# double125/MADTP

Measured on AMD Instinct MI355X. Metric: images/sec forward, BLIP-base NLVR2 p=0.5 b64; pruned-token index match, higher is better.
Workload: dtype bf16

## Files before the change

include/madtp_hip.h:

```cpp
#ifndef MADTP_HIP_H
#define MADTP_HIP_H

#include <stddef.h>
#include <stdint.h>

#ifdef __cplusplus
extern "C" {
#endif

#define MADTP_F32 0
#define MADTP_BF16 1
#define MADTP_F16S 2
#define MADTP_F16 3

#define MADTP_E_BADARG (-1)
#define MADTP_E_SHAPE (-2)
#define MADTP_E_DTYPE (-3)
#define MADTP_E_ALIGN (-4)
#define MADTP_E_BUSY (-5)
#define MADTP_E_RANGE (-6)

#define MADTP_ACT_NONE 0
#define MADTP_ACT_GELU_ERF 1
#define MADTP_ACT_QUICK_GELU 2
// ... 185 lines not shown
    const float* self_mask_qk;
    int ld_self_mask_qk;
} madtp_bert_layer_w;

size_t madtp_bert_layer_workspace(int B, int L, int Nk, int dim, int hidden, int heads, int dtype);

int madtp_bert_layer_attn(const madtp_bert_layer_w* w, const float* hidden, const float* mask2d, float* att, void* ws,
                          size_t ws_bytes, int B, int L, int Nk, const float* token_attn, int ldt_row, int ldt_batch, int K,
                          float temperature, float* score, float* threshold, int32_t* count, int32_t* kmax, void* stream);

int madtp_bert_layer_rest(const madtp_bert_layer_w* w, const float* att, const float* mask2d, float* y, float* mask_out,
                          void* ws, size_t ws_bytes, int B, int L, int k, const float* score, int64_t* indices,
                          int64_t* indices_sort, int cross_mode, const void* enc0, const void* enc1, int Nk,
                          const float* enc_mask0, const float* enc_mask1, void* stream);

int madtp_bert_layer(const madtp_bert_layer_w* w, const float* hidden, const float* mask2d, float* att, float* y,
                     float* mask_out, void* ws, size_t ws_bytes, int B, int L, int Nk, const float* token_attn, int ldt_row,
                     int ldt_batch, int K, float temperature, float* score, float* threshold, int32_t* count,
                     int64_t* indices, int64_t* indices_sort, int cross_mode, const void* enc0, const void* enc1,
                     const float* enc_mask0, const float* enc_mask1, const void* hidden_lp, void* y_lp, const void* kv_pre0,
                     const void* kv_pre1, const int32_t* kv_index, int kv_ld, int* k_out, int* k_used, void* stream);

typedef struct madtp_query_w {
    const void* sd_w;
    const void* sd_hi; const void* sd_lo; int split_dtype; float sd_scale;
    int K; float inv_sqrt_sd;
    float* att_ft;
    float* stats_ws;
} madtp_query_w;

typedef struct madtp_layer_io {
    float* logits;
    float* x_attn;
    float* y;
    void* y_lp;
    float* mask_out;
    float* score; float* threshold; int32_t* count;
    int64_t* indices; int64_t* indices_sort;
    int k_out, k_used, n_out;
} madtp_layer_io;

int madtp_vit_encoder(const madtp_vit_block_w* const* layers, int n_layers, const madtp_query_w* q, const float* x0,
                      madtp_layer_io* io, void* ws, size_t ws_bytes, int B, int N0, float temperature, void* stream);

int madtp_vit_encoder_async(const madtp_vit_block_w* const* layers, int n_layers, const madtp_query_w* q, const float* x0,
                            madtp_layer_io* io, void* ws, size_t ws_bytes, int B, int N0, float temperature, int32_t* dims_dev,
                            int32_t* dims_host, void* stream);

int madtp_bert_encoder(const madtp_bert_layer_w* const* layers, int n_layers, const madtp_query_w* q, const float* hidden0,
                       const void* hidden0_lp, const float* mask0, madtp_layer_io* io, void* ws, size_t ws_bytes, int B, int L0,
                       int Nk, float temperature, int cross_mode, const void* enc0, const void* enc1, const float* enc_mask0,
                       const float* enc_mask1, const void* const* kv_pre0, const void* const* kv_pre1, const int32_t* kv_index,
                       int kv_ld, void* stream);

int madtp_bert_encoder_async(const madtp_bert_layer_w* const* layers, int n_layers, const madtp_query_w* q, const float* hidden0,
                             const void* hidden0_lp, const float* mask0, madtp_layer_io* io, void* ws, size_t ws_bytes, int B, int L0,
                             int Nk, float temperature, int cross_mode, const void* enc0, const void* enc1, const float* enc_mask0,
                             const float* enc_mask1, const void* const* kv_pre0, const void* const* kv_pre1, const int32_t* kv_index,
                             int kv_ld, int32_t* dims_dev, int32_t* dims_host, void* stream);

int madtp_bert_decode_step(const madtp_bert_layer_w* const* layers, int n_layers, const float* x, void* kv_cache, int rows, int t,
                           int Lmax, const void* const* kv_pre, const int32_t* kv_index, int kv_ld, int Nk, int group, float* y,
                           void* ws, size_t ws_bytes, void* stream);
int madtp_kv_cache_reorder(const void* src, void* dst, const int64_t* beam_src, int n_layers, int rows, int Lmax, int t, int row_bytes,
                           void* stream);

int madtp_lm_loss(const float* logits, int ld, int rows_per_seq, int n_pred, int V, const int64_t* labels, int ld_labels,
                  float label_smoothing, float* loss, int B, void* stream);
int madtp_token_prob(const float* logits, int ld, int V, const int64_t* tok, int A, float* out, int Q, void* stream);
int madtp_beam_topk(const float* logits, int ld, int V, const float* beam_scores, int num_beams, int n_top, int suppress_token,
                    float* out_scores, int32_t* out_index, int B, void* stream);
int madtp_beam_topk_penalty(const float* logits, int ld, int V, const float* beam_scores, int num_beams, int n_top,
                            int suppress_token, const int64_t* prev_ids, int ld_prev, int cur_len, float repetition_penalty,
                            float* out_scores, int32_t* out_index, int B, void* stream);
int madtp_beam_update(const float* cand_scores, const int32_t* cand_index, int n_top, int V, const int64_t* ids_in, int64_t* ids_out,
                      int ld_ids, int cur_len, float* beam_scores, int64_t* beam_src, int32_t* hyp_n, int32_t* hyp_order,
                      double* hyp_score, int32_t* hyp_len, int64_t* hyp_tok, double* worst, int32_t* done, int32_t* err, double denom,
                      int num_beams, int eos_token, int pad_token, int early_stopping, int B, void* stream);
int madtp_sample_top_p(const float* logits, int ld, int V, const int64_t* prev_ids, int ld_prev, int cur_len, float repetition_penalty,
                       int suppress_token, int top_k, float top_p, const float* u, int64_t* out_token, float* out_prob, int B,
                       void* stream);


int madtp_transpose_pad(const float* src, int ld_src, int R, int C, float* dst, int ld_dst, int Rp, int Cp, void* stream);
int madtp_transpose_split(const float* src, int ld_src, int R, int C, void* dst, int Rp, int Cp, int weight_format,
                          float* colsum_out, float* colsum_ws, void* stream);
int madtp_weight_planes(const float* w, int ldw, int N, int K, float inv_scale, void* planes, int row0, void* planes_t, int Ntp, int col0,
                        void* stream);
int madtp_colsum(const float* dy, int ld, int M, int N, float* out, float* part_ws, void* stream);
int madtp_act_fwd_bwd(const float* u, const float* dg, float* g, float* du, size_t n, int act, void* stream);
int madtp_layernorm_bwd(const float* x, const float* gamma, const float* dy, const float* add, float* dx, float* dgamma,
                        float* dbeta, float* ws, int rows, int dim, float eps, void* stream);
int madtp_token_gather_bwd(const float* dy, const float* x, const int32_t* dst_pos, const float* merge_w, float* dx, float* dw,
                           int B, int N, int k, int dim, void* stream);
int madtp_token_score_bwd(const float* dw, const float* score, const int32_t* dst_pos, const float* merge_w,
                          const float* colsum_part, int n_row_tiles, const float* p0, const float* onorm,
                          const float* token_attn, int ldt_row, int ldt_batch, int K, float* da, float* dp0, float* dnrm_scale,
                          float* dtoken_attn, int B, int H, int N, void* stream);
size_t madtp_attention_bwd_cross_workspace(int B, int H, int Nq, int Nk);
int madtp_attention_bwd_cross(const float* q, int ldq, const float* k, const float* v, int ldkv, const float* key_mask,
                              const float* dout, int ldo, float* dq, int lddq, float* dk, float* dv, int lddkv, void* ws,
                              size_t ws_bytes, int B, int H, int Nq, int Nk, float scale, float p_drop,
                              unsigned long long seed, unsigned long long site, void* stream);

int madtp_dropout(const float* x, const float* residual, float* y, size_t n, size_t per_sample, float p, unsigned long long seed,
                  unsigned long long site, void* stream);
// ... 36 lines not shown
```

madtp_amd/bert.py:

```python
import json
import math
import os

import torch
import torch.nn as nn

from . import hip
from .runtime import autograd_precision as _autograd_precision, EncoderWeights, PreparedCache, param_epoch, own_modules, get_precision, encoder_call_preference, f32_ptr, attn_dtype, compute_dtype, dtype_code, lin_of, require_gpu, as_f32_contig, to_compute
from .utils import Query_model


class BertConfig:
    _defaults = dict(vocab_size=30522, hidden_size=768, num_hidden_layers=12, num_attention_heads=12,
                     intermediate_size=3072, hidden_act="gelu", hidden_dropout_prob=0.1,
                     attention_probs_dropout_prob=0.1, max_position_embeddings=512, type_vocab_size=2,
                     initializer_range=0.02, layer_norm_eps=1e-12, pad_token_id=0, position_embedding_type="absolute",
                     add_cross_attention=False, encoder_width=768, chunk_size_feed_forward=0, evaluate=True,
                     output_attentions=False, output_hidden_states=False, use_return_dict=True, is_decoder=False)

    def __init__(self, **kw):
        for k, v in {**self._defaults, **kw}.items():
            setattr(self, k, v)

    @classmethod
# ... 554 lines not shown
    def _enc_mask2d(m):
        if m is None:
            return None
        return as_f32_contig(m[:, 0, 0, :]) if m.dim() == 4 else as_f32_contig(m)

    def feed_forward_chunk(self, attention_output):
        raise NotImplementedError("fused into forward()")


class MedBertLayer(_BertLayerBase):
    variant = "med"

    def forward(self, hidden_states, attention_mask=None, head_mask=None, encoder_hidden_states=None,
                encoder_attention_mask=None, past_key_value=None, output_attentions=False, mode=None, space_dict=None,
                token_attn=None, reduce_num=0, temperature=0):
        return self._forward(hidden_states, attention_mask, head_mask, encoder_hidden_states, encoder_attention_mask,
                             past_key_value, output_attentions, mode, token_attn, temperature)


class NlvrBertLayer(_BertLayerBase):
    variant = "nlvr"

    def forward(self, hidden_states, attention_mask=None, space_dict=None, head_mask=None, encoder_hidden_states=None,
                encoder_attention_mask=None, past_key_value=None, output_attentions=False, mode=None, token_attn=None,
                reduce_num=0, temperature=0):
        return self._forward(hidden_states, attention_mask, head_mask, encoder_hidden_states, encoder_attention_mask,
                             past_key_value, output_attentions, mode, token_attn, temperature)


class _Out(tuple):

    def __new__(cls, last_hidden_state):
        o = super().__new__(cls, (last_hidden_state,))
        o.last_hidden_state = last_hidden_state
        o.past_key_values = None
        o.hidden_states = None
        o.attentions = None
        o.cross_attentions = None
        o.pooler_output = None
        return o


class _BertEncoderBase(nn.Module):
    layer_cls = MedBertLayer

    def __init__(self, config, sd_dim=768):
        super().__init__()
        self.config = config
        self.layer = nn.ModuleList([self.layer_cls(config, i) for i in range(config.num_hidden_layers)])
        self.gradient_checkpointing = False
        self.txt_query_model = Query_model(ft_dim=config.hidden_size, sd_dim=sd_dim, temperature=1,
                                           att_func_type='sparsemax', pool_type='max')
        self._cache = PreparedCache()

    def _run(self, hidden_states, attention_mask, space_dict, temperature, encoder_hidden_states, encoder_attention_mask,
             mode, always_query):
        sd_txt_ft_all = None
        cache = self.__dict__.pop("_kv_cache", None)
        if torch.is_grad_enabled() and _autograd_precision() and cache is None:
            encs = [] if encoder_hidden_states is None else (list(encoder_hidden_states) if isinstance(encoder_hidden_states, (list, tuple))
                                                              else [encoder_hidden_states])
            if (hidden_states.requires_grad or (space_dict is not None and space_dict.requires_grad)
                    or any(e.requires_grad for e in encs) or any(p.requires_grad for p in self.parameters())):
                from .backward import bert_encoder_forward_with_grad
                self.__dict__.pop("_prepared_weights", None)
                h, _, sd_all = bert_encoder_forward_with_grad(self, hidden_states, attention_mask, space_dict, temperature,
                                                              encoder_hidden_states, encoder_attention_mask, mode, always_query)
                return _Out(h), sd_all
        if (_use_encoder_call(hidden_states.shape[0], _ENCODER_CALL) and not _KV_AHEAD
                and all(type(l) is self.layer_cls for l in self.layer)):
            out = self._run_encoder_call(hidden_states, attention_mask, space_dict, temperature, encoder_hidden_states,
                                         encoder_attention_mask, mode, always_query, cache)
            if out is not None:
                return out
        defer = self.txt_query_model.deferred() if space_dict is not None else None
        reduce_num = int((hidden_states.shape[-2] - 1) // self.config.num_hidden_layers)
        ahead = None
        if cache is None and mode == 'multimodal' and encoder_hidden_states is not None and _KV_AHEAD:
            ahead = self._project_encoder_tokens(encoder_hidden_states)
        for i, layer_module in enumerate(self.layer):
            layer_module.__dict__.pop("_kv_pre", None)
            if cache is not None and mode == 'multimodal':
                layer_module._kv_pre = (cache.kv[i], cache.Nk, cache.index)
            elif ahead is not None:
                kvs, Nk, width = ahead
                layer_module._kv_pre = (tuple(kv[:, i * width:(i + 1) * width] for kv in kvs) if len(kvs) == 2
                                        else kvs[0][:, i * width:(i + 1) * width], Nk, None)
            token_attn = None
            if space_dict is not None or always_query:
                if space_dict is None:
                    raise TypeError("nlvr_encoder.BertEncoder calls txt_query_model unconditionally (:608): "
                                    "space_dict must be given")
                token_attn, sd_txt_ft_all, _ = self.txt_query_model(hidden_states[:, 1:, :], space_dict,
                                                                    return_token_att=True, temperature=temperature,
                                                                    acc_ft=sd_txt_ft_all, defer=defer)
            t = temperature if space_dict is not None else 0
            if self.layer_cls.variant == "nlvr":
                outs = layer_module(hidden_states, attention_mask, space_dict, None, encoder_hidden_states,
                                    encoder_attention_mask, None, False, mode=mode, token_attn=token_attn,
                                    reduce_num=reduce_num, temperature=t)
            else:
                outs = layer_module(hidden_states, attention_mask, None, encoder_hidden_states, encoder_attention_mask,
                                    None, False, mode=mode, space_dict=space_dict, token_attn=token_attn,
                                    reduce_num=reduce_num, temperature=t)
            hidden_states = outs[0]
            attention_mask = outs[-1]
        if defer is not None and defer.pairs:
            sd_txt_ft_all = defer.finish()
        return _Out(hidden_states), sd_txt_ft_all


    def _run_options(self, hidden_states, attention_mask, head_mask, encoder_hidden_states, encoder_attention_mask, past_key_values,
                     use_cache, output_attentions, output_hidden_states, mode, space_dict, temperature, always_query):
        all_hidden = () if output_hidden_states else None
        all_self = () if output_attentions else None
        all_cross = () if (output_attentions and mode == 'multimodal') else None
        next_cache = () if use_cache else None
        sd_txt_ft_all = None
        require_gpu(hidden_states, "hidden_states")
        for i, layer_module in enumerate(self.layer):
            layer_module.__dict__.pop("_kv_pre", None)
            if output_hidden_states:
                all_hidden = all_hidden + (hidden_states,)
            token_attn = None
            if space_dict is not None or always_query:
                if space_dict is None:
                    raise TypeError("nlvr_encoder.BertEncoder calls txt_query_model unconditionally (:608): space_dict must be given")
                token_attn, sd_txt_ft_all, _ = self.txt_query_model(hidden_states[:, 1:, :], space_dict, return_token_att=True,
                                                                    temperature=temperature, acc_ft=sd_txt_ft_all)
            t = temperature if space_dict is not None else 0
            lhm = head_mask[i] if head_mask is not None else None
            hm = layer_module._head_mask_vec(lhm, hidden_states.device) if lhm is not None else None
            outs = layer_module._forward_general(as_f32_contig(hidden_states), attention_mask, hm, encoder_hidden_states,
                                                 encoder_attention_mask, past_key_values[i] if past_key_values is not None else None,
                                                 bool(output_attentions), mode, token_attn, t)
            hidden_states, attention_mask = outs[0], outs[-1]
            if use_cache:
                next_cache = next_cache + (outs[-2],)
            if output_attentions:
                all_self = all_self + (outs[1],)
                if all_cross is not None:
                    all_cross = all_cross + ((outs[2] if len(outs) == 5 else tuple(outs[2:-2])),)
        if output_hidden_states:
            all_hidden = all_hidden + (hidden_states,)
        out = _Out(hidden_states)
        out.past_key_values, out.hidden_states, out.attentions, out.cross_attentions = next_cache, all_hidden, all_self, all_cross
        return out, sd_txt_ft_all

    def _apply(self, fn, recurse=True):
        self.__dict__.pop("_enc_weights", None)
        return super()._apply(fn, recurse)

    def _encoder_weights(self):
        ew = self.__dict__.get("_enc_weights")
        if ew is None:
            ew = self.__dict__["_enc_weights"] = EncoderWeights()
        return ew.get(list(self.layer))

    def prepare_encoder_call(self, batch=None):
        if (batch is None or _use_encoder_call(batch, _ENCODER_CALL)) and _ENCODER_CALL and not _KV_AHEAD \
                and all(type(l) is self.layer_cls for l in self.layer):
            self.__dict__["_prepared_weights"] = (param_epoch(), get_precision(), self._encoder_weights())

    def _run_encoder_call(self, hidden_states, attention_mask, space_dict, temperature, encoder_hidden_states,
                          encoder_attention_mask, mode, always_query, cache):
        require_gpu(hidden_states, "hidden_states")
        query = space_dict is not None or always_query
        if query and space_dict is None:
            raise TypeError("nlvr_encoder.BertEncoder calls txt_query_model unconditionally (:608): space_dict must be given")
        hidden = as_f32_contig(hidden_states)
        B, L, D = hidden.shape
        mask2d = None
        if attention_mask is not None:
            if attention_mask.dim() == 4 and attention_mask.shape[2] == L and L > 1:
                return None
            if attention_mask.dim() != 4 or attention_mask.shape[2] != 1:
                raise NotImplementedError("only padding masks [B,1,1,L] and decoder masks [B,1,L,L] are supported")
            mask2d = as_f32_contig(attention_mask[:, 0, 0, :])
        t = temperature if space_dict is not None else 0
        if t > 0 and mask2d is None:
            raise ValueError("attention_mask is required when temperature > 0 (med.py:424)")
        qargs, deferred = (None, False)
        if query:
            qargs, deferred = self.txt_query_model.encoder_args(space_dict, B, D, hidden.device)
            if qargs is None:
                return None
        l0 = self.layer[0]
        cross = mode == 'multimodal'
        enc0 = enc1 = em0 = em1 = None
        kv0 = kv1 = kv_index = None
        Nk = 0
        nlvr = self.layer_cls.variant == "nlvr"
        if cross and cache is not None:
            Nk, kv0, kv_index = cache.Nk, list(cache.kv), cache.index
            if nlvr:
                return None
        elif cross:
            assert encoder_hidden_states is not None, "encoder_hidden_states must be given for cross-attention layers"
            if nlvr:
                Nk = encoder_hidden_states[0].shape[1]
                enc0, enc1 = l0._enc_operand(encoder_hidden_states[0]), l0._enc_operand(encoder_hidden_states[1])
                em0, em1 = l0._enc_mask2d(encoder_attention_mask[0]), l0._enc_mask2d(encoder_attention_mask[1])
            else:
                Nk = encoder_hidden_states.shape[1]
                enc0 = l0._enc_operand(encoder_hidden_states)
        lp = getattr(hidden_states, "_madtp_lp", None)
        if lp is not None and (lp[1] != hidden._version or hidden is not hidden_states or lp[0].shape[:-1] != hidden.shape[:-1]
                               or compute_dtype() == torch.float32 or lp[0].dtype != compute_dtype()):
            lp = None
        ws = self.__dict__.pop("_prepared_weights", None)
        if ws is not None and ws[:2] == (param_epoch(), get_precision()):
            ws = ws[2]
        else:
            ws = self._encoder_weights()
        kv_ld = 0
        if kv0 is not None:
            for tns in kv0:
                if tns.stride(-1) != 1 or (kv_ld and kv_ld != tns.stride(0)):
                    raise RuntimeError("encoder_kv_cache tensors must be row-major with one common row stride")
                kv_ld = tns.stride(0)
        from . import vit as _vit
        sync_free = _vit._SYNC_FREE and query and t > 0 and hip.bert_encoder_sync_free_ok(B, L, Nk, True, qargs, mask2d)
        run = hip.bert_encoder(ws, hidden, lp[0] if lp else None, mask2d, qargs, t, cross, enc0, enc1, Nk, em0, em1,
                               kv_pre0=kv0, kv_pre1=kv1, kv_index=kv_index, kv_ld=kv_ld, sync_free=sync_free)
        for l, layer in enumerate(self.layer):
            layer.last_prune = run.info(l, t if query else 0)
            layer.__dict__.pop("_kv_pre", None)
        sd_txt_ft_all = None
        qm = self.txt_query_model
        if query and qm.compute_att_ft:
            if deferred:
                K = space_dict.shape[0]
                segs = []
                for l in range(len(self.layer)):
                    n_in = run.n_in(l)
                    xp = hidden.data_ptr() if l == 0 else run.ptr(l - 1, "y")
                    segs.append((run.ptr(l, "logits") + 128 * 4, xp + D * 4, n_in - 1, 128, n_in * 128, D, n_in * D))
                sd_txt_ft_all = hip.query_att_ft_multi_ptrs(segs, B, K, D, hidden.device, sd_dim=qm.att_dim, exact={"exact": True, "split": "split"}.get(deferred, False))
            else:
                sd_txt_ft_all = qargs["att_ft"]
        self._last_run = run
        out = run.output(len(self.layer) - 1)
        if run.lp_dtype is not None:
            nl = len(self.layer) - 1
            out._madtp_lp = (run.view(nl, "y_lp", run.lp_dtype, B, out.shape[1], (2 * D if run.lp_dtype == torch.float16 else D)),
                             out._version)
        return _Out(out), sd_txt_ft_all

    def _project_encoder_tokens(self, encoder_hidden_states):
        encs = list(encoder_hidden_states) if isinstance(encoder_hidden_states, (list, tuple)) else [encoder_hidden_states]
        if not all(getattr(l, "has_cross", hasattr(l, "crossattention")) for l in self.layer):
            return None
        kvs = []
        for br, enc in enumerate(encs):
            mods = []
            for l in self.layer:
                ca = l.crossattention
                sm = (ca.self0, ca.self1)[br] if ca.twin else ca.self
                mods += [sm.key, sm.value]
            lin = lin_of(self._cache, ("kv_all", br), mods)
            kvs.append(hip.gemm(self.layer[0]._enc_operand(enc), lin.w, lin.b, n=lin.n, out_dtype=attn_dtype()))
        return kvs, encs[0].shape[1], 2 * self.config.hidden_size


class MedBertEncoder(_BertEncoderBase):
    layer_cls = MedBertLayer

    def forward(self, hidden_states, attention_mask=None, head_mask=None, encoder_hidden_states=None,
                encoder_attention_mask=None, past_key_values=None, use_cache=None, output_attentions=False,
                output_hidden_states=False, return_dict=True, mode='multimodal', space_dict=None, temperature=0):
        if head_mask is not None or past_key_values is not None or use_cache or output_attentions or output_hidden_states:
            return self._run_options(hidden_states, attention_mask, head_mask, encoder_hidden_states, encoder_attention_mask,
                                     past_key_values, use_cache, output_attentions, output_hidden_states, mode, space_dict,
                                     temperature, always_query=False)
        return self._run(hidden_states, attention_mask, space_dict, temperature, encoder_hidden_states,
                         encoder_attention_mask, mode, always_query=False)


class NlvrBertEncoder(_BertEncoderBase):
    layer_cls = NlvrBertLayer

    def forward(self, hidden_states, attention_mask=None, space_dict=None, temperature=0, head_mask=None,
                encoder_hidden_states=None, encoder_attention_mask=None, past_key_values=None, use_cache=None,
                output_attentions=False, output_hidden_states=False, return_dict=True, mode='multimodal'):
        if head_mask is not None or past_key_values is not None or use_cache or output_attentions or output_hidden_states:
            return self._run_options(hidden_states, attention_mask, head_mask, encoder_hidden_states, encoder_attention_mask,
                                     past_key_values, use_cache, output_attentions, output_hidden_states, mode, space_dict,
                                     temperature, always_query=True)
        return self._run(hidden_states, attention_mask, space_dict, temperature, encoder_hidden_states,
                         encoder_attention_mask, mode, always_query=True)


class _BertModelBase(nn.Module):
    encoder_cls = MedBertEncoder

    def __init__(self, config, add_pooling_layer=True, sd_dim=768):
        super().__init__()
        if add_pooling_layer:
            raise NotImplementedError("BLIP builds its text encoders with add_pooling_layer=False")
        self.config = config
        self.embeddings = BertEmbeddings(config)
        self.encoder = self.encoder_cls(config, sd_dim)
        self.pooler = None
        if not getattr(config, "evaluate", True):
            self.apply(self._init_weights)

    def _init_weights(self, module):
        if isinstance(module, (nn.Linear, nn.Embedding)):
            module.weight.data.normal_(mean=0.0, std=self.config.initializer_range)
        elif isinstance(module, nn.LayerNorm):
            module.bias.data.zero_()
            module.weight.data.fill_(1.0)
        if isinstance(module, nn.Linear) and module.bias is not None:
            module.bias.data.zero_()

# ... 367 lines not shown
```

madtp_amd/csrc/layers.hip:

```cpp
#include "common.h"
#include "internal.h"
#include <stdlib.h>

namespace {

struct Carver {
    char* base; size_t off; size_t cap;
    void* take(size_t bytes) {
        off = (off + 255) & ~(size_t)255;
        void* p = base ? base + off : nullptr;
        off += bytes;
        return p;
    }
    bool fits() const { return !base || off <= cap; }
};

inline size_t esz_of(int dt) { return (dt == MADTP_BF16 || dt == MADTP_F16) ? 2 : 4; }
inline int pld(int dt, int ld) { return dt == MADTP_F16S ? 2 * ld : ld; }
inline int attn_dt(int dt) { return dt == MADTP_F16S ? MADTP_F32 : dt; }
inline int attn_io(int dt) { return dt == MADTP_F16S ? MADTP_F16S : dt; }
inline int slabs_of(int K, int dt) { return dt == MADTP_F32 ? K / 32 : K / 64; }

#define TRY(call)                  \
    do {                           \
// ... 797 lines not shown
                                       (const char*)k1 + (size_t)D * e, (kv_pre0 && kv_pre0[l]) ? kv_index : nullptr, v.cat,
                                       (char*)v.cat + (size_t)D * e, em0, em1, B, w->heads, L0, Nk, 2 * D, ldkv, ldkv, 2 * D, w->scale,
                                       attn_io(dt), 0, dl + DIMS_STRIDE, stream));
            const void* catc = v.cat;
            if (dt == MADTP_F16S) {
                TRY(madtp_i_split_f16((const float*)v.cat, 2 * D, v.mid, 4 * D, Mmax, 2 * D, m_out, stream));
                catc = v.mid;
            }
            TRY(lin_ln_dev(catc, 2 * D, w->cdense_fused, a32, w->fused_twin == 2 ? 1.f : 0.5f, w->ln_cross_g, w->ln_cross_b, v.att2,
                           lpm ? v.attc : nullptr, Mmax, dt, w->eps, v.part, m_out, stream));
            a32 = v.att2;
            ac = lpm ? (const void*)v.attc : (const void*)v.att2;
        } else if (cross == 1) {
            TRY(lin_dev(ac, D, w->cq[0], nullptr, 0, v.q, D, Mmax, dt, adt, MADTP_ACT_NONE, m_out, stream));
            const void* k0 = kv_pre0 ? kv_pre0[l] : nullptr;
            int ldkv = 2 * D;
            if (!k0) {
                if (!enc0) return MADTP_E_BADARG;
                TRY(lin(enc0, D, w->ckv[0], nullptr, 0, v.kv, 2 * D, B * Nk, dt, adt, MADTP_ACT_NONE, 1.f, stream));
                k0 = v.kv;
            } else if (kv_ld) ldkv = kv_ld;
            TRY(madtp_i_attention_cross(v.q, k0, (const char*)k0 + (size_t)D * e, (kv_pre0 && kv_pre0[l]) ? kv_index : nullptr, v.c0,
                                        w->variant_nlvr ? enc_mask0 : nullptr, B, w->heads, L0, Nk, D, ldkv, ldkv, D, w->scale, attn_io(dt),
                                        dl + DIMS_STRIDE, stream));
            const void* cc = v.c0;
            if (dt == MADTP_F16S) {
                TRY(madtp_i_split_f16((const float*)v.c0, D, v.mid, 2 * D, Mmax, D, m_out, stream));
                cc = v.mid;
            }
            TRY(lin_ln_dev(cc, D, w->cdense[0], a32, 1.f, w->ln_cross_g, w->ln_cross_b, v.att2, lpm ? v.attc : nullptr, Mmax, dt, w->eps,
                           v.part, m_out, stream));
            a32 = v.att2;
            ac = lpm ? (const void*)v.attc : (const void*)v.att2;
        }
        TRY(lin_dev(ac, D, w->inter, nullptr, 0, v.mid, w->inter.n, Mmax, dt, dt, MADTP_ACT_GELU_ERF, m_out, stream));
        TRY(lin_ln_dev(v.mid, w->inter.n, w->out, a32, 1.f, w->ln_out_g, w->ln_out_b, o.y, lpm ? o.y_lp : nullptr, Mmax, dt, w->eps, v.part,
                       m_out, stream));
        h = o.y;
        h_lp = lpm ? o.y_lp : nullptr;
        mask = o.mask_out;
    }
    he = hipMemcpyAsync(dims_host, dims_dev, nrec * sizeof(int32_t), hipMemcpyDeviceToHost, s);
    if (he == hipSuccess) he = hipStreamSynchronize(s);
    if (he != hipSuccess) return (int)he;
    for (int l = 0; l < n_layers; ++l) {
        io[l].k_out = dims_host[l * DIMS_STRIDE + 1];
        io[l].k_used = dims_host[l * DIMS_STRIDE + 2];
        io[l].n_out = dims_host[l * DIMS_STRIDE + 3];
    }
    const int* rf = madtp_internal_range_flag();
    return (rf && *(const volatile int*)rf) ? MADTP_E_RANGE : 0;
}

extern "C" int madtp_bert_encoder(const madtp_bert_layer_w* const* layers, int n_layers, const madtp_query_w* q, const float* hidden0,
                                  const void* hidden0_lp, const float* mask0, madtp_layer_io* io, void* ws, size_t ws_bytes, int B,
                                  int L0, int Nk, float temperature, int cross_mode, const void* enc0, const void* enc1,
                                  const float* enc_mask0, const float* enc_mask1, const void* const* kv_pre0,
                                  const void* const* kv_pre1, const int32_t* kv_index, int kv_ld, void* stream) {
    if (!layers || !io || !hidden0 || n_layers <= 0 || B <= 0 || L0 <= 0) return MADTP_E_BADARG;
    const float* h = hidden0;
    const void* h_lp = hidden0_lp;
    const float* mask = mask0;
    int L = L0;
    const bool prune = q && temperature > 0.f;
    const int kp = q ? (q->K + 127) / 128 * 128 : 0;
    for (int l = 0; l < n_layers; ++l) {
        madtp_layer_io& o = io[l];
        const madtp_bert_layer_w* w = layers[l];
        if (!w || !o.x_attn || !o.y) return MADTP_E_BADARG;
        if (q) {
            if (!o.logits) return MADTP_E_BADARG;
            TRY(query_step(q, h, o.logits, l, B, L, w->dim, stream));
        }
        int k_out = 0, k_used = 0;
        const void* kv0 = kv_pre0 ? kv_pre0[l] : nullptr;
        const void* kv1 = kv_pre1 ? kv_pre1[l] : nullptr;
        if (prune)
            TRY(madtp_bert_layer(w, h, mask, o.x_attn, o.y, o.mask_out, ws, ws_bytes, B, L, Nk, o.logits + kp, kp, L * kp, q->K,
                                 temperature, o.score, o.threshold, o.count, o.indices, o.indices_sort, cross_mode, enc0, enc1,
                                 enc_mask0, enc_mask1, h_lp, o.y_lp, kv0, kv1, kv_index, kv_ld, &k_out, &k_used, stream));
        else
            TRY(madtp_bert_layer(w, h, mask, o.x_attn, o.y, nullptr, ws, ws_bytes, B, L, Nk, nullptr, 0, 0, 0, 0.f, nullptr, nullptr,
                                 nullptr, nullptr, nullptr, cross_mode, enc0, enc1, enc_mask0, enc_mask1, h_lp, o.y_lp, kv0, kv1,
                                 kv_index, kv_ld, &k_out, &k_used, stream));
        if (k_used > 0) {
            L = k_used + 2;
            if (mask) mask = o.mask_out;
        }
        o.k_out = k_out; o.k_used = k_used; o.n_out = L;
        h = o.y;
        h_lp = o.y_lp;
    }
    return 0;
}
```

madtp_amd/hip.py:

```python
import ctypes
import os
from ctypes import c_float, c_int, c_size_t, c_void_p

import torch

F32, BF16, F16S, F16 = 0, 1, 2, 3
ACT_NONE, ACT_GELU, ACT_QUICK_GELU, ACT_RELU = 0, 1, 2, 3
ABI_VERSION = 31

_HERE = os.path.dirname(os.path.abspath(__file__))
LIB_PATH = os.path.join(_HERE, "lib", "libmadtp_hip.so")

_SIGS = {
    "madtp_abi_version": (c_int, []),
    "madtp_strerror": (ctypes.c_char_p, [c_int]),
    "madtp_profile_begin": (c_int, []),
    "madtp_profile_end": (c_int, [ctypes.c_char_p, c_int]),
    "madtp_gemm": (c_int, [c_void_p] * 5 + [c_int] * 7 + [c_int, c_int, c_int, c_float, c_float, c_void_p]),
    "madtp_gemm_set_config": (c_int, [c_int]),
    "madtp_gemm_plan": (c_int, [c_int] * 11 + [c_void_p, c_void_p, c_int]),
    "madtp_stream_create_cumask": (c_int, [c_void_p, c_void_p, c_int]),
    "madtp_stream_set_sched": (c_int, [c_void_p, c_int, c_float, c_int]),
    "madtp_stream_get_sched": (c_int, [c_void_p, c_void_p, c_void_p, c_void_p]),
    "madtp_stream_destroy": (c_int, [c_void_p]),
# ... 2 lines not shown
    "madtp_splitk_ln": (c_int, [c_void_p, c_int, c_void_p, c_void_p, c_void_p, c_void_p, c_void_p, c_void_p, c_int, c_int, c_int,
                                c_float, c_float, c_float, c_void_p]),
    "madtp_layernorm": (c_int, [c_void_p] * 5 + [c_int, c_int, c_int, c_float, c_void_p]),
    "madtp_patchify": (c_int, [c_void_p, c_void_p, c_int, c_int, c_int, c_int, c_void_p]),
    "madtp_assemble_tokens": (c_int, [c_void_p] * 4 + [c_int, c_int, c_int, c_void_p]),
    "madtp_bert_embed": (c_int, [c_void_p] * 7 + [c_int, c_int, c_int, c_int, c_float, c_void_p]),
    "madtp_attention": (c_int, [c_void_p] * 8 + [c_int] * 8 + [c_float, c_int, c_void_p]),
    "madtp_attention_qk_mask": (c_int, [c_void_p] * 6 + [c_int] + [c_void_p] * 3 + [c_int] * 8 + [c_float, c_int, c_void_p]),
    "madtp_token_score": (c_int, [c_void_p, c_int, c_void_p, c_void_p, c_void_p, c_int, c_int, c_int, c_float]
                          + [c_void_p] * 4 + [c_int, c_int, c_int, c_void_p]),
    "madtp_token_select": (c_int, [c_void_p, c_int] + [c_void_p] * 4 + [c_int, c_int, c_void_p]),
    "madtp_token_gather": (c_int, [c_void_p] * 4 + [c_int] * 4 + [c_void_p]),
    "madtp_token_gather_ln": (c_int, [c_void_p] * 4 + [c_int] * 4 + [c_void_p, c_void_p, c_float, c_void_p, c_void_p, c_int, c_void_p]),
    "madtp_mask_gather": (c_int, [c_void_p, c_void_p, c_int, c_void_p, c_int, c_void_p, c_int, c_int, c_int, c_void_p]),
    "madtp_query_att_ft": (c_int, [c_void_p, c_int, c_int, c_int, c_void_p, c_int, c_int, c_void_p, c_float, c_int,
                                   c_int, c_int, c_int, c_int, c_void_p, c_void_p]),
    "madtp_align_logits": (c_int, [c_void_p, c_void_p, c_void_p, c_void_p, c_int, c_int, c_int, c_float, c_void_p]),
    "madtp_vector_gather": (c_int, [c_void_p, c_void_p, c_void_p, c_int, c_int, c_int, c_int, c_void_p]),
    "madtp_vit_block_workspace": (c_size_t, [c_int] * 6),
    "madtp_vit_block_attn": (c_int, [c_void_p, c_void_p, c_void_p, c_void_p, c_size_t, c_int, c_int, c_void_p, c_int, c_int,
                                     c_int, c_float, c_void_p, c_void_p, c_void_p, c_void_p, c_void_p]),
    "madtp_vit_block_mlp": (c_int, [c_void_p, c_void_p, c_void_p, c_void_p, c_size_t, c_int, c_int, c_int, c_void_p,
                                    c_void_p, c_void_p, c_void_p]),
    "madtp_query_model": (c_int, [c_void_p, c_void_p, c_void_p, c_void_p, c_int, c_float, c_int, c_void_p, c_void_p, c_void_p,
                                  c_int, c_float, c_int, c_int, c_int, c_void_p]),
    "madtp_bert_layer_workspace": (c_size_t, [c_int] * 7),
    "madtp_bert_layer_attn": (c_int, [c_void_p, c_void_p, c_void_p, c_void_p, c_void_p, c_size_t, c_int, c_int, c_int,
                                      c_void_p, c_int, c_int, c_int, c_float, c_void_p, c_void_p, c_void_p, c_void_p,
                                      c_void_p]),
    "madtp_bert_layer_rest": (c_int, [c_void_p, c_void_p, c_void_p, c_void_p, c_void_p, c_void_p, c_size_t, c_int, c_int,
                                      c_int, c_void_p, c_void_p, c_void_p, c_int, c_void_p, c_void_p, c_int, c_void_p,
                                      c_void_p, c_void_p]),
    "madtp_token_score_sync": (c_int, [c_void_p, c_int, c_void_p, c_void_p, c_void_p, c_int, c_int, c_int, c_float]
                               + [c_void_p] * 4 + [c_int, c_int, c_int, c_void_p]),
    "madtp_token_score_publish": (c_int, [c_void_p, c_int, c_void_p, c_void_p, c_void_p, c_int, c_int, c_int, c_float]
                                  + [c_void_p] * 3 + [c_int, c_int, c_int, c_void_p, c_void_p]),
    "madtp_token_score_wait": (c_int, [c_int, c_void_p, c_int, c_void_p, c_void_p]),
    "madtp_attention_indexed": (c_int, [c_void_p] * 9 + [c_int] * 8 + [c_float, c_int, c_void_p]),
    "madtp_vit_block": (c_int, [c_void_p] * 5 + [c_size_t, c_int, c_int, c_void_p, c_int, c_int, c_int, c_float]
                        + [c_void_p] * 7 + [c_void_p]),
    "madtp_vit_block_keep": (c_int, [c_void_p] * 5 + [c_size_t, c_int, c_int, c_void_p, c_int, c_int, c_int, c_float]
                             + [c_void_p] * 5 + [c_int] + [c_void_p] * 2 + [c_void_p]),
    "madtp_bert_layer": (c_int, [c_void_p] * 7 + [c_size_t, c_int, c_int, c_int, c_void_p, c_int, c_int, c_int, c_float]
                         + [c_void_p] * 5 + [c_int] + [c_void_p] * 9 + [c_int] + [c_void_p] * 3),
    "madtp_vit_encoder": (c_int, [c_void_p, c_int, c_void_p, c_void_p, c_void_p, c_void_p, c_size_t, c_int, c_int, c_float, c_void_p]),
    "madtp_vit_encoder_async": (c_int, [c_void_p, c_int, c_void_p, c_void_p, c_void_p, c_void_p, c_size_t, c_int, c_int, c_float, c_void_p,
                                         c_void_p, c_void_p]),
    "madtp_bert_encoder": (c_int, [c_void_p, c_int, c_void_p, c_void_p, c_void_p, c_void_p, c_void_p, c_void_p, c_size_t, c_int, c_int,
                                   c_int, c_float, c_int, c_void_p, c_void_p, c_void_p, c_void_p, c_void_p, c_void_p, c_void_p, c_int,
                                   c_void_p]),
    "madtp_bert_encoder_async": (c_int, [c_void_p, c_int, c_void_p, c_void_p, c_void_p, c_void_p, c_void_p, c_void_p, c_size_t, c_int, c_int,
                                         c_int, c_float, c_int, c_void_p, c_void_p, c_void_p, c_void_p, c_void_p, c_void_p, c_void_p, c_int,
                                         c_void_p, c_void_p, c_void_p]),
    "madtp_bert_decode_step": (c_int, [c_void_p, c_int, c_void_p, c_void_p, c_int, c_int, c_int, c_void_p, c_void_p, c_int, c_int, c_int,
                                       c_void_p, c_void_p, c_size_t, c_void_p]),
    "madtp_kv_cache_reorder": (c_int, [c_void_p, c_void_p, c_void_p, c_int, c_int, c_int, c_int, c_int, c_void_p]),
    "madtp_sample_top_p": (c_int, [c_void_p, c_int, c_int, c_void_p, c_int, c_int, c_float, c_int, c_int, c_float, c_void_p, c_void_p, c_void_p,
                                   c_int, c_void_p]),
    "madtp_add_scale": (c_int, [c_void_p, c_void_p, c_void_p, c_float, c_size_t, c_void_p]),
    "madtp_gemm_pair": (c_int, [c_void_p] * 8 + [c_int] * 8 + [c_float, c_float, c_void_p]),
    "madtp_attention_pair": (c_int, [c_void_p] * 11 + [c_int] * 8 + [c_float, c_int, c_void_p]),
    "madtp_query_att_ft_multi": (c_int, [c_void_p, c_int, c_int, c_void_p, c_void_p, c_float, c_int, c_int, c_int, c_void_p]),
    "madtp_query_att_ft_multi_split": (c_int, [c_void_p, c_int, c_int, c_void_p, c_void_p, c_float, c_int, c_int, c_int, c_void_p]),
    "madtp_cast_bf16": (c_int, [c_void_p, c_void_p, c_size_t, c_void_p]),
    "madtp_cast_lp": (c_int, [c_void_p, c_void_p, c_size_t, c_int, c_float, c_void_p]),
    "madtp_range_status": (c_int, [c_int, c_void_p]),
    "madtp_split_f16": (c_int, [c_void_p, c_int, c_void_p, c_int, c_int, c_int, c_void_p]),
    "madtp_split_f16_weight": (c_int, [c_void_p, c_int, c_void_p, c_int, c_int, c_float, c_void_p]),
    "madtp_lm_loss": (c_int, [c_void_p, c_int, c_int, c_int, c_int, c_void_p, c_int, c_float, c_void_p, c_int, c_void_p]),
    "madtp_token_prob": (c_int, [c_void_p, c_int, c_int, c_void_p, c_int, c_void_p, c_int, c_void_p]),
    "madtp_beam_topk": (c_int, [c_void_p, c_int, c_int, c_void_p, c_int, c_int, c_int, c_void_p, c_void_p, c_int, c_void_p]),
    "madtp_beam_topk_penalty": (c_int, [c_void_p, c_int, c_int, c_void_p, c_int, c_int, c_int, c_void_p, c_int, c_int, c_float, c_void_p,
                                         c_void_p, c_int, c_void_p]),
    "madtp_transpose_pad": (c_int, [c_void_p, c_int, c_int, c_int, c_void_p, c_int, c_int, c_int, c_void_p]),
    "madtp_gemm_splitk_pp": (c_int, [c_void_p, c_void_p, c_void_p, c_int, c_int, c_int, c_int, c_int, c_int, c_float, c_void_p]),
    "madtp_splitk_sum": (c_int, [c_void_p, c_int, c_size_t, c_void_p, c_void_p]),
    "madtp_beam_update": (c_int, [c_void_p, c_void_p, c_int, c_int, c_void_p, c_void_p, c_int, c_int, c_void_p, c_void_p, c_void_p, c_void_p,
                                  c_void_p, c_void_p, c_void_p, c_void_p, c_void_p, c_void_p, ctypes.c_double, c_int, c_int, c_int, c_int, c_int,
                                  c_void_p]),
    "madtp_weight_planes": (c_int, [c_void_p, c_int, c_int, c_int, c_float, c_void_p, c_int, c_void_p, c_int, c_int, c_void_p]),
    "madtp_transpose_split": (c_int, [c_void_p, c_int, c_int, c_int, c_void_p, c_int, c_int, c_int, c_void_p, c_void_p, c_void_p]),
    "madtp_colsum": (c_int, [c_void_p, c_int, c_int, c_int, c_void_p, c_void_p, c_void_p]),
    "madtp_act_fwd_bwd": (c_int, [c_void_p, c_void_p, c_void_p, c_void_p, c_size_t, c_int, c_void_p]),
    "madtp_layernorm_bwd": (c_int, [c_void_p] * 8 + [c_int, c_int, c_float, c_void_p]),
    "madtp_itc_workspace": (c_size_t, [c_int, c_int, c_int]),
    "madtp_itc_loss": (c_int, [c_void_p] * 7 + [c_float] + [c_void_p] * 4 + [c_size_t, c_int, c_int, c_int, c_void_p]),
    "madtp_ema_blocks": (c_int, [ctypes.c_int64]),
    "madtp_ema_update": (c_int, [c_void_p, c_int, c_int, c_float, c_float, c_void_p]),
    "madtp_itm_negatives": (c_int, [c_void_p] * 10 + [c_int, c_int, c_int, c_void_p]),
    "madtp_token_gather_bwd": (c_int, [c_void_p] * 6 + [c_int] * 4 + [c_void_p]),
    "madtp_token_score_bwd": (c_int, [c_void_p] * 5 + [c_int, c_void_p, c_void_p, c_void_p, c_int, c_int, c_int] + [c_void_p] * 4
                              + [c_int, c_int, c_int, c_void_p]),
    "madtp_attention_probs": (c_int, [c_void_p, c_void_p, c_int, c_void_p, c_void_p, c_int, c_int, c_int, c_float, c_void_p]),
    "madtp_attention_probs_x": (c_int, [c_void_p, c_void_p, c_int, c_int, c_void_p, c_void_p, c_int, c_void_p, c_int, c_int, c_int, c_int,
                                        c_float, c_void_p]),
    "madtp_att_ft_bwd": (c_int, [c_void_p, c_void_p, c_void_p, c_float, c_void_p, c_void_p, c_void_p, c_int, c_int, c_int, c_int, c_void_p]),
    "madtp_attention_bwd_workspace": (c_size_t, [c_int, c_int, c_int]),
    "madtp_attention_bwd_cross_workspace": (c_size_t, [c_int, c_int, c_int, c_int]),
    "madtp_attention_bwd_cross": (c_int, [c_void_p, c_int, c_void_p, c_void_p, c_int, c_void_p, c_void_p, c_int, c_void_p, c_int, c_void_p,
                                          c_void_p, c_int, c_void_p, c_size_t, c_int, c_int, c_int, c_int, c_float, c_float, ctypes.c_uint64,
                                          ctypes.c_uint64, c_void_p]),
    "madtp_attention_bwd": (c_int, [c_void_p, c_void_p, c_void_p, c_int, c_void_p, c_void_p, c_int, c_void_p, c_int, c_void_p, c_int] + [c_void_p] * 6
                            + [c_int, c_void_p, c_size_t, c_void_p, c_int, c_int, c_int, c_float, c_float, ctypes.c_uint64, ctypes.c_uint64, c_void_p]),
    "madtp_dropout": (c_int, [c_void_p, c_void_p, c_void_p, c_size_t, c_size_t, c_float, ctypes.c_uint64, ctypes.c_uint64, c_void_p]),
    "madtp_attention_train": (c_int, [c_void_p, c_int, c_void_p, c_void_p, c_int, c_void_p, c_void_p, c_int, c_void_p, c_void_p, c_int, c_void_p,
                                      c_void_p, c_void_p, c_int, c_int, c_int, c_int, c_float, c_float, ctypes.c_uint64, ctypes.c_uint64, c_void_p]),
# ... 539 lines not shown
    amax = float(w.abs().max())
    s = 0
    if amax > 0 and amax == amax and amax != float("inf"):
        import math
        s = max(-100, min(100, 14 - math.ceil(math.log2(amax))))
    dst = cast_bf16(w, scale=2.0 ** s)
    dst._madtp_w_scale = float(2.0 ** -s)
    return dst


def range_status(reset=True):
    return int(load().madtp_range_status(1 if reset else 0, _stream()))


def split_f16(src):
    _req(src, torch.float32, "src")
    K = src.shape[-1]
    rows = src.numel() // K
    dst = torch.empty(tuple(src.shape[:-1]) + (2 * K,), device=src.device, dtype=torch.float16)
    _check(load().madtp_split_f16(_p(src), K, _p(dst), 2 * K, rows, K, _stream()), "madtp_split_f16")
    return dst


def split_f16_weight(w, log2_scale=None):
    _req(w, torch.float32, "w")
    n, K = w.shape
    s = 0
    amax = float(w.abs().max()) if log2_scale is None else 0.0
    if log2_scale is not None:
        s = int(log2_scale)
    elif amax > 0 and amax == amax and amax != float("inf"):
        import math
        s = 14 - math.ceil(math.log2(amax))
        s = max(-100, min(100, s))
    dst = torch.empty((n, 2 * K), device=w.device, dtype=torch.float16)
    _check(load().madtp_split_f16_weight(_p(w), K, _p(dst), n, K, float(2.0 ** s), _stream()), "madtp_split_f16_weight")
    dst._madtp_w_scale = float(2.0 ** -s)
    dst._madtp_log2_scale = s
    return dst


def vector_gather(vectors, indices):
    _req(vectors, torch.float32, "vectors"); _req(indices, torch.int64, "indices")
    B, L, D = vectors.shape
    K = indices.shape[1]
    out = torch.empty((B, K, D), device=vectors.device, dtype=torch.float32)
    _check(load().madtp_vector_gather(_p(vectors), _p(indices), _p(out), B, L, K, D, _stream()), "madtp_vector_gather")
    return out


_WS = {}


def workspace(nbytes, device):
    key = (device.type, device.index, torch.cuda.current_stream(device).cuda_stream if device.type == "cuda" else 0)
    ws = _WS.get(key)
    if ws is None or ws.numel() < nbytes:
        ws = torch.empty(int(nbytes * 1.25) + 4096, dtype=torch.uint8, device=device)
        _WS[key] = ws
    return ws


def prune_outputs(B, n, device):
    return (torch.empty((B, n), device=device, dtype=torch.float32), torch.empty((B,), device=device, dtype=torch.float32),
            torch.empty((B,), device=device, dtype=torch.int32), None)


def token_score_sync(side, token_attn, temperature, B, H, N):
    cs, p0, on = side
    tp, ldr, ldb, K = _ta_view(token_attn)
    score, thr, count, _ = prune_outputs(B, N - 1, token_attn.device)
    k = ctypes.c_int32(-1)
    _check(load().madtp_token_score_sync(_p(cs), cs.shape[1], _p(p0), _p(on), tp, ldr, ldb, K, float(temperature), _p(score),
                                         _p(thr), _p(count), ctypes.byref(k), B, H, N, _stream()), "madtp_token_score_sync")
    return score, thr, count, k.value


def batch_max_count(count):
    return int(count.cpu().max())


def _carve(buf, *shape):
    n = 1
    for d in shape:
        n *= d
    return buf.view(-1)[:n].view(*shape)


def vit_block(wstruct, x, token_attn, temperature, max_keep=0):
    B, N, D = x.shape
    lib = load()
    nbytes = lib.madtp_vit_block_workspace(B, N, wstruct.dim, wstruct.fc1.n, wstruct.heads, wstruct.dtype)
    ws = workspace(nbytes, x.device)
    x_attn = torch.empty_like(x)
    ybuf = torch.empty_like(x)
    k_out, k_used = ctypes.c_int(0), ctypes.c_int(0)
    if temperature > 0:
        tp, ldr, ldb, K = _ta_view(token_attn)
        score, thr, count, _ = prune_outputs(B, N - 1, x.device)
        idx = torch.empty((B, N - 1), device=x.device, dtype=torch.int64)
        idx_sort = torch.empty((B, N - 1), device=x.device, dtype=torch.int64)
        _check(lib.madtp_vit_block_keep(ctypes.byref(wstruct), _p(x), _p(x_attn), _p(ybuf), _p(ws), ws.numel(), B, N, tp, ldr, ldb,
                                        K, float(temperature), _p(score), _p(thr), _p(count), _p(idx), _p(idx_sort), int(max_keep),
                                        ctypes.byref(k_out), ctypes.byref(k_used), _stream()), "madtp_vit_block_keep")
        info = {"k": k_out.value, "score": score, "threshold": thr, "count": count, "pruned": False, "indices": None,
                "indices_sort": None}
        if k_used.value > 0:
            k = k_used.value
# ... 476 lines not shown
        raise ValueError("bert_decode_step: kv_index must hold one entry per group of rows")
    _check(lib.madtp_bert_decode_step(arr, L, _p(x), _p(kv_cache), rows, int(t), kv_cache.shape[2], kv, _p(kv_index), int(kv_ld), int(Nk),
                                      int(group), _p(y), _p(ws), ws.numel(), _stream()), "madtp_bert_decode_step")
    return y


def kv_cache_reorder(src, dst, beam_src, t):
    L, rows, Lmax, W = src.shape
    _check(load().madtp_kv_cache_reorder(_p(src), _p(dst), _p(beam_src), L, rows, Lmax, int(t), W * src.element_size(), _stream()),
           "madtp_kv_cache_reorder")


def bert_encoder_sync_free_ok(B, L, Nk, prune, qargs, mask2d):
    return bool(prune and qargs is not None and qargs.get("att_ft") is None and mask2d is not None and B * L < 4096
                and 3 <= L <= 256 and Nk <= 256)


def bert_encoder(weights, hidden, hidden_lp, mask2d, qargs, temperature, cross_mode, enc0, enc1, Nk, enc_mask0, enc_mask1,
                 kv_pre0=None, kv_pre1=None, kv_index=None, kv_ld=0, sync_free=False):
    B, Lq, D = hidden.shape
    lib = load()
    wstructs, arr = weights
    L = len(wstructs)
    w0 = wstructs[0]
    nbytes = lib.madtp_bert_layer_workspace(B, Lq, Nk, w0.dim, w0.inter.n, w0.heads, w0.dtype)
    ws = workspace(nbytes, hidden.device)
    prune = qargs is not None and temperature > 0
    lp_dtype = None if w0.dtype == F32 else (torch.float16 if w0.dtype == F16S else torch.bfloat16)
    run = EncoderRun(L, B, Lq, D, hidden.device, qargs is not None, prune, mask2d is not None and prune, lp_dtype)
    q = _query_w(qargs)
    kv0 = (c_void_p * L)(*[_p(t) for t in kv_pre0]) if kv_pre0 is not None else None
    kv1 = (c_void_p * L)(*[_p(t) for t in kv_pre1]) if kv_pre1 is not None else None
    if sync_free:
        if not bert_encoder_sync_free_ok(B, Lq, Nk, prune, qargs, mask2d):
            raise RuntimeError("sync-free encoder call: needs pruning with a deferred att_ft and a padding mask, B * L < 4096 rows, "
                               "L <= 256 and <= 256 keys")
        dims_dev = torch.empty(((L + 2) * 4,), device=hidden.device, dtype=torch.int32)
        dims_host = (ctypes.c_int32 * ((L + 1) * 4))()
        _check(lib.madtp_bert_encoder_async(arr, L, ctypes.byref(q), _p(hidden), _p(hidden_lp), _p(mask2d), run.io_ptr, _p(ws), ws.numel(),
                                            B, Lq, Nk, float(temperature), int(cross_mode), _p(enc0), _p(enc1), _p(enc_mask0),
                                            _p(enc_mask1), kv0, kv1, _p(kv_index), int(kv_ld), _p(dims_dev), ctypes.addressof(dims_host),
                                            _stream()), "madtp_bert_encoder_async")
        run.keep = (hidden, hidden_lp, mask2d, wstructs, qargs, enc0, enc1, enc_mask0, enc_mask1, kv_pre0, kv_pre1, kv_index, dims_dev,
                    dims_host)
        return run
    _check(lib.madtp_bert_encoder(arr, L, ctypes.byref(q) if q is not None else None, _p(hidden), _p(hidden_lp), _p(mask2d), run.io_ptr,
                                  _p(ws), ws.numel(), B, Lq, Nk, float(temperature if prune else 0.0), int(cross_mode), _p(enc0),
                                  _p(enc1), _p(enc_mask0), _p(enc_mask1), kv0, kv1, _p(kv_index), int(kv_ld), _stream()),
           "madtp_bert_encoder")
    run.keep = (hidden, hidden_lp, mask2d, wstructs, qargs, enc0, enc1, enc_mask0, enc_mask1, kv_pre0, kv_pre1, kv_index)
    return run


def _gpu_f32(t, name, dims):
    if not (t.is_cuda and t.dtype == torch.float32 and t.dim() == dims and t.is_contiguous()):
        raise RuntimeError(f"{name}: a contiguous GPU f32 tensor of {dims} dimensions is required")


def _gpu_i64(t, name):
    if not (t.is_cuda and t.dtype == torch.int64 and t.is_contiguous()):
        raise RuntimeError(f"{name}: a contiguous GPU int64 tensor is required")


def itc_loss(q, q_m, keys_batch, queue, idx, idx_queue, temp, alpha):
    for t, n in ((q, "q"), (q_m, "q_m"), (keys_batch, "keys_batch"), (queue, "queue")):
        _gpu_f32(t, f"itc_loss: {n}", 2)
    _gpu_i64(idx, "itc_loss: idx")
    _gpu_i64(idx_queue, "itc_loss: idx_queue")
    if not (temp.is_cuda and temp.dtype == torch.float32 and temp.numel() == 1):
        raise RuntimeError("itc_loss: temp must be a one-element GPU f32 tensor")
    B, D = q.shape
    Q = queue.shape[1]
    if q_m.shape != (B, D) or keys_batch.shape != (B, D) or queue.shape[0] != D or idx.numel() != B or idx_queue.numel() != Q:
        raise RuntimeError("itc_loss: shapes disagree")
    lib = load()
    ws_bytes = int(lib.madtp_itc_workspace(B, D, Q))
    ws = torch.empty(max(ws_bytes, 4) // 4 + 1, dtype=torch.float32, device=q.device)
    loss = torch.empty(B, dtype=torch.float32, device=q.device)
    dq = torch.empty(B, D, dtype=torch.float32, device=q.device)
    dtemp = torch.empty(1, dtype=torch.float32, device=q.device)
    _check(lib.madtp_itc_loss(_p(q), _p(q_m), _p(keys_batch), _p(queue) if Q else 0, _p(idx), _p(idx_queue) if Q else 0, _p(temp),
                              float(alpha), _p(loss), _p(dq), _p(dtemp), _p(ws), ws.numel() * 4, B, D, Q, _stream()), "madtp_itc_loss")
    return loss, dq, dtemp


class EmaTable:

    def __init__(self):
        self._ptrs, self._table, self._blocks = None, None, 0

    def update(self, pairs, m):
        ptrs = [t.data_ptr() for pair in pairs for t in pair]
        lib = load()
        if ptrs != self._ptrs:
            for pm, p in pairs:
                if not (pm.is_cuda and pm.dtype == torch.float32 and pm.is_contiguous() and p.shape == pm.shape
                        and p.dtype == pm.dtype and p.is_contiguous() and p.device == pm.device):
                    raise RuntimeError("ema_update: every pair must be two contiguous GPU f32 tensors of one shape")
            first, nb = [], 0
            for pm, _ in pairs:
                first.append(nb)
                nb += int(lib.madtp_ema_blocks(pm.numel()))
            rows = [ptrs[0::2], ptrs[1::2], [pm.numel() for pm, _ in pairs], first]
            self._table = torch.tensor(rows, dtype=torch.int64).to(pairs[0][0].device)
            self._ptrs, self._blocks = ptrs, nb
            self._n = len(pairs)
# ... 30 lines not shown
```

Before: 26800.

## Precompute all-layer cross-attention K/V in one GEMM for bf16 encoder call

Adds a native entry point that projects encoder (image) tokens through the concatenated key/value weights of every layer in one GEMM (or a paired GEMM for twin branches), writing into a dedicated workspace pool. The fused single-call encoder path is now allowed with KV-ahead in bf16, and the precomputed per-layer K/V slices are passed in as kv_pre. This replaces the per-layer cross-attention K/V projections with one large GEMM. It adds a second workspace pool and is only active when the KV-ahead flag or the per-module attribute asks for it.

```diff
diff --git a/include/madtp_hip.h b/include/madtp_hip.h
--- a/include/madtp_hip.h
+++ b/include/madtp_hip.h
@@ -261,6 +261,9 @@
                        int Nk, float temperature, int cross_mode, const void* enc0, const void* enc1, const float* enc_mask0,
                        const float* enc_mask1, const void* const* kv_pre0, const void* const* kv_pre1, const int32_t* kv_index,
                        int kv_ld, void* stream);
+
+int madtp_bert_cross_kv(const madtp_lin* kv_all0, const madtp_lin* kv_all1, const void* enc0, const void* enc1, void* out0,
+                        void* out1, int rows, int n_layers, int dim, int dtype, int launches, void* stream);
 
 int madtp_bert_encoder_async(const madtp_bert_layer_w* const* layers, int n_layers, const madtp_query_w* q, const float* hidden0,
                              const void* hidden0_lp, const float* mask0, madtp_layer_io* io, void* ws, size_t ws_bytes, int B, int L0,
diff --git a/madtp_amd/bert.py b/madtp_amd/bert.py
--- a/madtp_amd/bert.py
+++ b/madtp_amd/bert.py
@@ -630,6 +630,13 @@
         self.txt_query_model = Query_model(ft_dim=config.hidden_size, sd_dim=sd_dim, temperature=1,
                                            att_func_type='sparsemax', pool_type='max')
         self._cache = PreparedCache()
+        self.kv_ahead = None
+
+    def _kv_ahead_wanted(self, cache, mode, encoder_hidden_states):
+        if cache is not None or mode != 'multimodal' or encoder_hidden_states is None:
+            return False
+        want = self.__dict__.get("kv_ahead")
+        return _KV_AHEAD if want is None else bool(want)
 
     def _run(self, hidden_states, attention_mask, space_dict, temperature, encoder_hidden_states, encoder_attention_mask,
              mode, always_query):
@@ -645,7 +652,7 @@
                 h, _, sd_all = bert_encoder_forward_with_grad(self, hidden_states, attention_mask, space_dict, temperature,
                                                               encoder_hidden_states, encoder_attention_mask, mode, always_query)
                 return _Out(h), sd_all
-        if (_use_encoder_call(hidden_states.shape[0], _ENCODER_CALL) and not _KV_AHEAD
+        if (_use_encoder_call(hidden_states.shape[0], _ENCODER_CALL) and not (_KV_AHEAD and compute_dtype() != torch.bfloat16)
                 and all(type(l) is self.layer_cls for l in self.layer)):
             out = self._run_encoder_call(hidden_states, attention_mask, space_dict, temperature, encoder_hidden_states,
                                          encoder_attention_mask, mode, always_query, cache)
@@ -654,7 +661,7 @@
         defer = self.txt_query_model.deferred() if space_dict is not None else None
         reduce_num = int((hidden_states.shape[-2] - 1) // self.config.num_hidden_layers)
         ahead = None
-        if cache is None and mode == 'multimodal' and encoder_hidden_states is not None and _KV_AHEAD:
+        if self._kv_ahead_wanted(cache, mode, encoder_hidden_states):
             ahead = self._project_encoder_tokens(encoder_hidden_states)
         for i, layer_module in enumerate(self.layer):
             layer_module.__dict__.pop("_kv_pre", None)
@@ -736,7 +743,8 @@
         return ew.get(list(self.layer))
 
     def prepare_encoder_call(self, batch=None):
-        if (batch is None or _use_encoder_call(batch, _ENCODER_CALL)) and _ENCODER_CALL and not _KV_AHEAD \
+        if (batch is None or _use_encoder_call(batch, _ENCODER_CALL)) and _ENCODER_CALL \
+                and not (_KV_AHEAD and compute_dtype() != torch.bfloat16) \
                 and all(type(l) is self.layer_cls for l in self.layer):
             self.__dict__["_prepared_weights"] = (param_epoch(), get_precision(), self._encoder_weights())
 
@@ -791,6 +799,13 @@
             ws = ws[2]
         else:
             ws = self._encoder_weights()
+        if compute_dtype() == torch.bfloat16 and self._kv_ahead_wanted(cache, mode, encoder_hidden_states):
+            ahead = self._project_encoder_tokens(encoder_hidden_states, weights_sig=self.__dict__["_enc_weights"].sig
+                                                 if "_enc_weights" in self.__dict__ else None)
+            if ahead is not None:
+                kvs, _, width = ahead
+                kv0 = [kvs[0][:, i * width:(i + 1) * width] for i in range(len(self.layer))]
+                kv1 = [kvs[1][:, i * width:(i + 1) * width] for i in range(len(self.layer))] if len(kvs) == 2 else None
         kv_ld = 0
         if kv0 is not None:
             for tns in kv0:
@@ -825,20 +840,33 @@
                              out._version)
         return _Out(out), sd_txt_ft_all
 
-    def _project_encoder_tokens(self, encoder_hidden_states):
+    def _project_encoder_tokens(self, encoder_hidden_states, weights_sig=None):
         encs = list(encoder_hidden_states) if isinstance(encoder_hidden_states, (list, tuple)) else [encoder_hidden_states]
         if not all(getattr(l, "has_cross", hasattr(l, "crossattention")) for l in self.layer):
             return None
-        kvs = []
-        for br, enc in enumerate(encs):
-            mods = []
-            for l in self.layer:
-                ca = l.crossattention
-                sm = (ca.self0, ca.self1)[br] if ca.twin else ca.self
-                mods += [sm.key, sm.value]
-            lin = lin_of(self._cache, ("kv_all", br), mods)
-            kvs.append(hip.gemm(self.layer[0]._enc_operand(enc), lin.w, lin.b, n=lin.n, out_dtype=attn_dtype()))
+        if len(encs) != (2 if self.layer[0].crossattention.twin else 1):
+            return None
+        hit = self.__dict__.get("_kv_all")
+        if weights_sig is not None and hit is not None and hit[0] is weights_sig:
+            lins = hit[1]
+        else:
+            lins = [self._kv_all_linear(br) for br in range(len(encs))]
+            if weights_sig is not None:
+                self.__dict__["_kv_all"] = (weights_sig, lins)
+        ops = [self.layer[0]._enc_operand(enc) for enc in encs]
+        if compute_dtype() == torch.bfloat16:
+            kvs, _ = hip.bert_cross_kv(lins, ops, len(self.layer), self.config.hidden_size)
+        else:
+            kvs = [hip.gemm(op, lin.w, lin.b, n=lin.n, out_dtype=attn_dtype()) for op, lin in zip(ops, lins)]
         return kvs, encs[0].shape[1], 2 * self.config.hidden_size
+
+    def _kv_all_linear(self, br):
+        mods = []
+        for l in self.layer:
+            ca = l.crossattention
+            sm = (ca.self0, ca.self1)[br] if ca.twin else ca.self
+            mods += [sm.key, sm.value]
+        return lin_of(self._cache, ("kv_all", br), mods)
 
 
 class MedBertEncoder(_BertEncoderBase):
diff --git a/madtp_amd/csrc/layers.hip b/madtp_amd/csrc/layers.hip
--- a/madtp_amd/csrc/layers.hip
+++ b/madtp_amd/csrc/layers.hip
@@ -873,6 +873,26 @@
     return (rf && *(const volatile int*)rf) ? MADTP_E_RANGE : 0;
 }
 
+extern "C" int madtp_bert_cross_kv(const madtp_lin* kv_all0, const madtp_lin* kv_all1, const void* enc0, const void* enc1, void* out0,
+                                   void* out1, int rows, int n_layers, int dim, int dtype, int launches, void* stream) {
+    if (!kv_all0 || !enc0 || !out0 || rows <= 0 || n_layers <= 0 || dim <= 0 || launches < 0 || launches > 2) return MADTP_E_BADARG;
+    if ((kv_all1 != nullptr) != (enc1 != nullptr) || (kv_all1 != nullptr) != (out1 != nullptr)) return MADTP_E_BADARG;
+    if (dtype != MADTP_BF16 && dtype != MADTP_F16) return MADTP_E_DTYPE;
+    const long long n_all = (long long)n_layers * 2 * dim;
+    const int K = kv_all0->k;
+    if (n_all > (1 << 20) || kv_all0->n != (int)n_all || K <= 0 || !kv_all0->w) return MADTP_E_SHAPE;
+    if (kv_all1 && (kv_all1->n != (int)n_all || kv_all1->k != K || !kv_all1->w || (!kv_all0->b) != (!kv_all1->b))) return MADTP_E_SHAPE;
+    const int N = (int)n_all;
+    if (kv_all1 && launches == 1)
+        return madtp_gemm_pair(enc0, enc1, kv_all0->w, kv_all1->w, kv_all0->b, kv_all1->b, out0, out1, rows, N, K, K, K, N, dtype, dtype,
+                               kv_all0->w_scale, kv_all1->w_scale, stream);
+    TRY(madtp_gemm(enc0, kv_all0->w, kv_all0->b, nullptr, out0, rows, N, K, K, K, N, 0, dtype, dtype, MADTP_ACT_NONE, kv_all0->w_scale,
+                   1.f, stream));
+    if (!kv_all1) return 0;
+    return madtp_gemm(enc1, kv_all1->w, kv_all1->b, nullptr, out1, rows, N, K, K, K, N, 0, dtype, dtype, MADTP_ACT_NONE, kv_all1->w_scale,
+                      1.f, stream);
+}
+
 extern "C" int madtp_bert_encoder(const madtp_bert_layer_w* const* layers, int n_layers, const madtp_query_w* q, const float* hidden0,
                                   const void* hidden0_lp, const float* mask0, madtp_layer_io* io, void* ws, size_t ws_bytes, int B,
                                   int L0, int Nk, float temperature, int cross_mode, const void* enc0, const void* enc1,
diff --git a/madtp_amd/hip.py b/madtp_amd/hip.py
--- a/madtp_amd/hip.py
+++ b/madtp_amd/hip.py
@@ -78,6 +78,7 @@
     "madtp_bert_encoder_async": (c_int, [c_void_p, c_int, c_void_p, c_void_p, c_void_p, c_void_p, c_void_p, c_void_p, c_size_t, c_int, c_int,
                                          c_int, c_float, c_int, c_void_p, c_void_p, c_void_p, c_void_p, c_void_p, c_void_p, c_void_p, c_int,
                                          c_void_p, c_void_p, c_void_p]),
+    "madtp_bert_cross_kv": (c_int, [c_void_p] * 6 + [c_int] * 5 + [c_void_p]),
     "madtp_bert_decode_step": (c_int, [c_void_p, c_int, c_void_p, c_void_p, c_int, c_int, c_int, c_void_p, c_void_p, c_int, c_int, c_int,
                                        c_void_p, c_void_p, c_size_t, c_void_p]),
     "madtp_kv_cache_reorder": (c_int, [c_void_p, c_void_p, c_void_p, c_int, c_int, c_int, c_int, c_int, c_void_p]),
@@ -723,8 +724,8 @@
 _WS = {}
 
 
-def workspace(nbytes, device):
-    key = (device.type, device.index, torch.cuda.current_stream(device).cuda_stream if device.type == "cuda" else 0)
+def workspace(nbytes, device, pool="layers"):
+    key = (device.type, device.index, torch.cuda.current_stream(device).cuda_stream if device.type == "cuda" else 0, pool)
     ws = _WS.get(key)
     if ws is None or ws.numel() < nbytes:
         ws = torch.empty(int(nbytes * 1.25) + 4096, dtype=torch.uint8, device=device)
@@ -1307,6 +1308,30 @@
     return run
 
 
+def cross_kv_layout(n_layers, D, branches, rows, esz=2):
+    kv_ld = n_layers * 2 * D
+    per = (rows * kv_ld * esz + 255) // 256 * 256
+    return kv_ld, [l * 2 * D for l in range(n_layers)], [br * per for br in range(branches)]
+
+
+def bert_cross_kv(lins, encs, n_layers, D, launches=0):
+    rows = encs[0].shape[0]
+    for t in encs:
+        _req(t, torch.bfloat16, "encoder tokens")
+        if t.dim() != 2 or t.shape != encs[0].shape:
+            raise RuntimeError("bert_cross_kv: encoder tokens must be [rows, width] of one shape")
+    kv_ld, _, offs = cross_kv_layout(n_layers, D, len(encs), rows)
+    ws = workspace(offs[-1] + rows * kv_ld * 2 + 256, encs[0].device, pool="cross_kv")
+    base = (-ws.data_ptr()) % 256
+    outs = [ws[base + o:base + o + rows * kv_ld * 2].view(torch.bfloat16).view(rows, kv_ld) for o in offs]
+    st = [lin_struct(l) for l in lins]
+    two = len(encs) == 2
+    _check(load().madtp_bert_cross_kv(ctypes.byref(st[0]), ctypes.byref(st[1]) if two else None, _p(encs[0]), _p(encs[1]) if two else 0,
+                                      _p(outs[0]), _p(outs[1]) if two else 0, rows, n_layers, D, _dt(encs[0]), int(launches), _stream()),
+           "madtp_bert_cross_kv")
+    return outs, kv_ld
+
+
 def _gpu_f32(t, name, dims):
     if not (t.is_cuda and t.dtype == torch.float32 and t.dim() == dims and t.is_contiguous()):
         raise RuntimeError(f"{name}: a contiguous GPU f32 tensor of {dims} dimensions is required")
```

Result: slower. 26260 (-2.0%).
